# yxgeee/OpenIBL

Measured on NVIDIA H100. Metric: images_per_sec_extraction, higher is better.
Workload: dtype f32 (bf16x3 split on wgmma, fp32 accumulate)

## Files before the change

include/iblb200.h:

```cpp
#ifndef IBLB200_H_
#define IBLB200_H_

#include <stddef.h>
#include <stdint.h>

#ifdef __cplusplus
extern "C" {
#endif

#define IBLB200_ABI_VERSION 1

typedef enum ibl_status {
  IBL_OK = 0,
  IBL_ERR_BAD_ARG = 1,
  IBL_ERR_NOT_READY = 2,
  IBL_ERR_CUDA = 3,
  IBL_ERR_NO_DEVICE = 4,
  IBL_ERR_OOM = 5,
  IBL_ERR_UNSUPPORTED = 6
} ibl_status;

typedef struct ibl_engine ibl_engine;

#define IBL_OUT_VLAD 0x1u
// ... 91 lines not shown
                void* stream);

int ibl_debug_dist_flagged(ibl_engine* e, int* count, void* stream);
int ibl_debug_dist_path(ibl_engine* e, int* path);
int ibl_debug_knn_flagged(ibl_engine* e, int* count, void* stream);
int ibl_debug_rerank_workspace_bytes(ibl_engine* e, uint64_t* bytes);
int ibl_selftest_tc(ibl_engine* e, float* max_rel_err);

int ibl_debug_conv3x3(ibl_engine* e, const float* x_nhwc, int N, int H, int W, int cin,
                      const float* w_oihw, const float* bias, int cout, int relu, int pool, int mode,
                      int bn_override, float* y_nhwc, void* stream);

int ibl_debug_gemm_tn(ibl_engine* e, const float* A, const float* B, float* C, void* stream);
int ibl_debug_umma_strided(ibl_engine* e, const void* A, int rows, const void* B, int s0, int group_rows,
                           int base_mode, float* D, void* stream);
int ibl_debug_time_layer(ibl_engine* e, int layer, const float* x, int N, int H, int W, int bn_override,
                         int reps, float* ms_out);

#ifdef __cplusplus
}
#endif
#endif
```

openibl_b200/_cabi.py:

```python
from __future__ import annotations

import ctypes
import os
from ctypes import POINTER, c_char_p, c_double, c_float, c_int, c_int64, c_uint, c_uint64, c_void_p

_HERE = os.path.dirname(os.path.abspath(__file__))
LIB_PATH = os.path.join(_HERE, "lib", "libiblb200.so")

IBL_OK = 0
STATUS_NAMES = {0: "IBL_OK", 1: "IBL_ERR_BAD_ARG", 2: "IBL_ERR_NOT_READY", 3: "IBL_ERR_CUDA",
                4: "IBL_ERR_NO_DEVICE", 5: "IBL_ERR_OOM", 6: "IBL_ERR_UNSUPPORTED"}
OUT_VLAD, OUT_PCA, OUT_POOL = 0x1, 0x2, 0x4
CONV_SIMT_FP32, CONV_TC_BF16X3 = 0, 1

_P = c_void_p
SIGNATURES = {
    "ibl_abi_version": (c_int, []),
    "ibl_status_string": (c_char_p, [c_int]),
    "ibl_last_error": (c_char_p, []),
    "ibl_engine_create": (c_int, [c_int, POINTER(c_void_p)]),
    "ibl_engine_destroy": (c_int, [_P]),
    "ibl_engine_set_conv_mode": (c_int, [_P, c_int]),
    "ibl_engine_set_gemm_mode": (c_int, [_P, c_int]),
    "ibl_engine_get_conv_mode": (c_int, [_P, POINTER(c_int)]),
# ... 26 lines not shown
    "ibl_argsort_rows": (c_int, [_P, _P, c_int, c_int, _P, _P]),
    "ibl_topk_merge": (c_int, [_P, _P, _P, c_int, c_int, c_int, c_int, _P, _P, _P]),
    "ibl_l2dist_topk_host": (c_int, [_P, _P, c_int, _P, c_int, c_int, c_int, _P, _P, _P]),
    "ibl_knn_rowmax": (c_int, [_P, _P, c_int, c_int, c_int, c_int, c_int, _P, _P, _P, _P]),
    "ibl_rerank_topk": (c_int, [_P, _P, c_int, c_int, c_int, _P, _P, c_int, _P, c_int, c_int, c_float, _P, c_int,
                                c_int, _P, _P, _P]),
    "ibl_rerank_dense": (c_int, [_P, _P, _P, _P, c_int, c_int, c_int, c_int, c_double, _P, _P]),
    "ibl_debug_rerank_workspace_bytes": (c_int, [_P, POINTER(c_uint64)]),
    "ibl_debug_knn_flagged": (c_int, [_P, POINTER(c_int), _P]),
    "ibl_gemm_nt": (c_int, [_P, _P, c_int, _P, c_int, c_int, c_float, _P, c_int, _P]),
    "ibl_debug_dist_flagged": (c_int, [_P, POINTER(c_int), _P]),
    "ibl_debug_dist_path": (c_int, [_P, POINTER(c_int)]),
    "ibl_selftest_tc": (c_int, [_P, POINTER(c_float)]),
    "ibl_debug_gemm_tn": (c_int, [_P, _P, _P, _P, _P]),
    "ibl_debug_umma_strided": (c_int, [_P, _P, c_int, _P, c_int, c_int, c_int, _P, _P]),
    "ibl_debug_time_layer": (c_int, [_P, c_int, _P, c_int, c_int, c_int, c_int, c_int, POINTER(c_float)]),
    "ibl_debug_conv3x3": (c_int, [_P, _P, c_int, c_int, c_int, c_int, _P, _P, c_int, c_int, c_int, c_int,
                                  c_int, _P, _P]),
}

_lib = None


class IblError(RuntimeError):
    def __init__(self, status: int, where: str, detail: str):
        self.status = status
        super().__init__(f"{where}: {STATUS_NAMES.get(status, status)}: {detail}")


def load(build_if_missing: bool = True) -> ctypes.CDLL:
# ... 23 lines not shown
```

openibl_b200/csrc/common.cuh:

```cuda
#pragma once
#include <cuda_runtime.h>
#include <cuda_bf16.h>
#include <stdint.h>
#include <stdio.h>
#include <atomic>
#include <string>

#include "../../include/iblb200.h"

namespace ibl {

void set_last_error(const std::string& s);

#define IBL_CUDA_OK(expr)                                                          \
  do {                                                                             \
    cudaError_t _e = (expr);                                                       \
    if (_e != cudaSuccess) {                                                       \
      ::ibl::set_last_error(std::string(#expr) + ": " + cudaGetErrorString(_e) +   \
                            " (" __FILE__ ":" + std::to_string(__LINE__) + ")");   \
      return IBL_ERR_CUDA;                                                         \
    }                                                                              \
  } while (0)

#define IBL_RET(expr)                 \
// ... 72 lines not shown
                              const int* kk_h, int ksize_h, const int* bounds_v, const int* kk_v, int ksize_v,
                              uint8_t* tmp, uint8_t* out, cudaStream_t s, uint64_t* launches);
int launch_repack_weights_dgrad(const float* w_tck, int cout, int cin, __nv_bfloat16* w_hi, __nv_bfloat16* w_lo,
                                cudaStream_t s);
int launch_relu_mask_planes(const float* g, const float* y, size_t n, bool relu, __nv_bfloat16* hi, __nv_bfloat16* lo,
                            cudaStream_t s);
int launch_maxpool2x2_bwd(const float* x, const float* gy, int N, int H, int W, int C, float* gx, cudaStream_t s);
int wgrad_tc_splits(int N, int H, int W, int cin, int cout);
int launch_conv_wgrad_tc(const __nv_bfloat16* g_hi, const __nv_bfloat16* g_lo, const __nv_bfloat16* x_hi,
                         const __nv_bfloat16* x_lo, int N, int H, int W, int cin, int cout, float* part, int splits,
                         float* bpart, float* dw_oihw, float* db, cudaStream_t s);
int launch_conv1_1_wgrad(const float* x_nchw, const __nv_bfloat16* g_hi, const __nv_bfloat16* g_lo, int N, int H, int W,
                         float* part, float* dw_oihw, float* db, cudaStream_t s);
int launch_conv1_1_tc(const float* x_nchw, const float* w_oihw, const float* bias, int N, int H, int W,
                      __nv_bfloat16* y_hi, __nv_bfloat16* y_lo, cudaStream_t s);
int debug_gmma_strided(const void* A, int rows, const void* B, int s0, int group_rows, int base_mode, float* D,
                       cudaStream_t s);
int debug_gemm_tn(const float* A, const float* B, float* C, cudaStream_t s);
int netvlad_tc_units(int B, int S);
int launch_netvlad_tc(const __nv_bfloat16* x_hi, const __nv_bfloat16* x_lo, int B, int S,
                      const __nv_bfloat16* w_hi, const __nv_bfloat16* w_lo, const float* ssq, int ssq_parts,
                      const float* cent, bool normalize_input, float* part, float* asum_part, int* ticket,
                      float* vlad_raw, float* vlad_norm, cudaStream_t s);
int launch_global_maxpool_planes(const __nv_bfloat16* hi, const __nv_bfloat16* lo, int N, int S, int C, float* y,
                                 cudaStream_t s);

int dist_top16_max_runs(int n_valid);
int launch_dist_top16_tc(const __nv_bfloat16* q_hi, const __nv_bfloat16* q_lo, const float* qn, int m,
                         const __nv_bfloat16* d_hi, const __nv_bfloat16* d_lo, const float* dn, int n,
                         int n_valid, int K, float* cand_d, long long* cand_i, int max_runs, int* runs_out,
                         cudaStream_t s);
int launch_dist_dense_tc(const __nv_bfloat16* q_hi, const __nv_bfloat16* q_lo, const float* qn, int m,
// ... 72 lines not shown
```

openibl_b200/csrc/engine.cu:

```cuda
#include <stdlib.h>

#include <mutex>
#include <new>
#include <vector>

#include "common.cuh"

namespace ibl {

static thread_local std::string g_last_error;
void set_last_error(const std::string& s) { g_last_error = s; }
void tc_set_bn_override(int bn);

static const ConvLayer kVgg16[13] = {
    {3, 64, true, false},    {64, 64, true, true},
    {64, 128, true, false},  {128, 128, true, true},
    {128, 256, true, false}, {256, 256, true, false}, {256, 256, true, true},
    {256, 512, true, false}, {512, 512, true, false}, {512, 512, true, true},
    {512, 512, true, false}, {512, 512, true, false}, {512, 512, false, false}
};

struct DevBuf {
  void* p = nullptr;
  size_t cap = 0;
// ... 1185 lines not shown
  return rc;
}

int ibl_debug_gemm_tn(ibl_engine* e, const float* A, const float* B, float* C, void* stream) {
  IBL_REQUIRE(e && A && B && C, "null argument");
  DeviceGuard g(e->device);
  e->launches += 3;
  return debug_gemm_tn(A, B, C, S(stream));
}

int ibl_debug_umma_strided(ibl_engine* e, const void* A, int rows, const void* B, int s0, int group_rows,
                            int base_mode, float* D, void* stream) {
  IBL_REQUIRE(e && A && B && D, "null argument");
  DeviceGuard g(e->device);
  e->launches += 1;
  return debug_gmma_strided(A, rows, B, s0, group_rows, base_mode, D, S(stream));
}

int ibl_debug_time_layer(ibl_engine* e, int layer, const float* x, int N, int H, int W, int bn_override,
                         int reps, float* ms_out) {
  IBL_REQUIRE(e && x && ms_out && layer >= 0 && layer <= 12 && reps >= 1, "bad argument");
  if (!e->vgg_ready) { set_last_error("ibl_engine_set_vgg16 was not called"); return IBL_ERR_NOT_READY; }
  DeviceGuard g(e->device);
  const ConvLayer& L = kVgg16[layer];
  const size_t in_e = (size_t)N * H * W * L.cin;
  const int oh = L.pool ? H / 2 : H, ow = L.pool ? W / 2 : W;
  const size_t out_e = (size_t)N * oh * ow * L.cout;
  IBL_RET(e->act[0].ensure((in_e > out_e ? in_e : out_e) * 4));
  IBL_RET(e->act[1].ensure((in_e > out_e ? in_e : out_e) * 4));
  cudaEvent_t e0, e1;
  IBL_CUDA_OK(cudaEventCreate(&e0));
  IBL_CUDA_OK(cudaEventCreate(&e1));
  __nv_bfloat16* ih = e->act[0].as<__nv_bfloat16>();
  __nv_bfloat16* oh_ = e->act[1].as<__nv_bfloat16>();
  int rc = IBL_OK;
  if (layer > 0) rc = launch_f32_to_planes(x, in_e, ih, ih + in_e, nullptr);
  tc_set_bn_override(bn_override);
  for (int r = -1; r < reps && rc == IBL_OK; ++r) {
    if (r == 0) cudaEventRecord(e0, nullptr);
    if (layer == 0)
      rc = launch_conv1_1_tc(x, e->w0_oihw, e->conv[0].bias, N, H, W, oh_, oh_ + out_e, nullptr);
    else
      rc = launch_conv3x3_tc(ih, ih + in_e, e->conv[layer], N, H, W, L.cin, L.cout, L.relu, L.pool,
                             layer == 12 ? nullptr : oh_, layer == 12 ? nullptr : oh_ + out_e,
                             layer == 12 ? e->act[1].as<float>() : nullptr, nullptr);
  }
  tc_set_bn_override(0);
  cudaEventRecord(e1, nullptr);
  cudaError_t ce = cudaEventSynchronize(e1);
  float ms = 0.f;
  cudaEventElapsedTime(&ms, e0, e1);
  cudaEventDestroy(e0);
  cudaEventDestroy(e1);
  if (rc == IBL_OK && ce != cudaSuccess) { set_last_error(cudaGetErrorString(ce)); return IBL_ERR_CUDA; }
  *ms_out = ms / reps;
// ... 6 lines not shown
```

openibl_b200/csrc/tc_common.cuh:

```cuda
#pragma once
#include <cuda.h>
#include <cuda_runtime.h>
#include <stdint.h>

#include "wgmma.cuh"

namespace ibl {
namespace tc {

__device__ __forceinline__ uint32_t smem_u32(const void* p) {
  return static_cast<uint32_t>(__cvta_generic_to_shared(p));
}

__device__ __forceinline__ uint32_t warp_uniform(uint32_t v) { return __reduce_or_sync(0xffffffffu, v); }

__device__ __forceinline__ bool elect_one() {
  uint32_t pred;
  asm volatile(
      "{\n\t"
      ".reg .pred p;\n\t"
      "elect.sync _|p, 0xffffffff;\n\t"
      "selp.u32 %0, 1, 0, p;\n\t"
      "}"
      : "=r"(pred));
// ... 161 lines not shown
}
__device__ __forceinline__ uint64_t gmma_desc_mnmajor_sw128(uint32_t smem_addr, uint32_t lbo_bytes) {
  uint64_t d = 0;
  d |= (uint64_t)((smem_addr >> 4) & 0x3fffu);
  d |= (uint64_t)((lbo_bytes >> 4) & 0x3fffu) << 16;
  d |= (uint64_t)(1024u >> 4) << 32;
  d |= (uint64_t)1 << 62;
  return d;
}

__device__ __forceinline__ void wgmma_fence() { asm volatile("wgmma.fence.sync.aligned;" ::: "memory"); }
__device__ __forceinline__ void wgmma_commit() { asm volatile("wgmma.commit_group.sync.aligned;" ::: "memory"); }
template <int N>
__device__ __forceinline__ void wgmma_wait() { asm volatile("wgmma.wait_group.sync.aligned %0;" ::"n"(N) : "memory"); }

__device__ __forceinline__ void wg_sync() { asm volatile("bar.sync 1, 128;" ::: "memory"); }

template <int N>
struct Acc128 {
  float h[2][N / 2];
  template <bool F16 = false, int TA = 0, int TB = 0>
  __device__ __forceinline__ void mma(uint64_t a0, uint64_t a1, uint64_t b, uint32_t accumulate) {
    Wgmma<N, F16, TA, TB>::mma(h[0], a0, b, accumulate);
    Wgmma<N, F16, TA, TB>::mma(h[1], a1, b, accumulate);
  }
  __device__ __forceinline__ void fence_operands() {
#pragma unroll
    for (int j = 0; j < 2; ++j)
#pragma unroll
      for (int i = 0; i < N / 2; ++i) asm volatile("" : "+f"(h[j][i])::"memory");
  }
  __device__ __forceinline__ void rows32(int ch, float* stg, uint32_t (&raw)[32]) const;
};
constexpr int ACC_STG_PITCH = 36;
constexpr int ACC_STG_BYTES = 128 * ACC_STG_PITCH * 4;

template <int N>
__device__ __forceinline__ void Acc128<N>::rows32(int ch, float* stg, uint32_t (&raw)[32]) const {
  const int t = threadIdx.x & 127, w = t >> 5, l = t & 31;
  wg_sync();
#pragma unroll
  for (int j = 0; j < 2; ++j)
#pragma unroll
    for (int i = 0; i < 4; ++i) {
      const int r = 64 * j + 16 * w + (l >> 2), c = 8 * i + 2 * (l & 3);
      const float* f = &h[j][4 * (4 * ch + i)];
      *reinterpret_cast<float2*>(stg + r * ACC_STG_PITCH + c) = make_float2(f[0], f[1]);
      *reinterpret_cast<float2*>(stg + (r + 8) * ACC_STG_PITCH + c) = make_float2(f[2], f[3]);
    }
  wg_sync();
#pragma unroll
  for (int i = 0; i < 8; ++i) {
    const float4 v = *reinterpret_cast<const float4*>(stg + t * ACC_STG_PITCH + 4 * i);
    raw[4 * i] = __float_as_uint(v.x); raw[4 * i + 1] = __float_as_uint(v.y);
    raw[4 * i + 2] = __float_as_uint(v.z); raw[4 * i + 3] = __float_as_uint(v.w);
  }
}

typedef CUresult (*EncodeTiledFn)(CUtensorMap*, CUtensorMapDataType, cuuint32_t, void*,
                                  const cuuint64_t*, const cuuint64_t*, const cuuint32_t*,
                                  const cuuint32_t*, CUtensorMapInterleave, CUtensorMapSwizzle,
                                  CUtensorMapL2promotion, CUtensorMapFloatOOBfill);
EncodeTiledFn get_encode_tiled();

int make_tmap(CUtensorMap* out, CUtensorMapDataType dt, int rank, const void* base,
// ... 5 lines not shown
```

openibl_b200/csrc/tc_conv.cu:

```cuda
#include "common.cuh"
#include "tc_common.cuh"

namespace ibl {

using namespace tc;

namespace tc {
EncodeTiledFn get_encode_tiled() {
  static const EncodeTiledFn fn = []() -> EncodeTiledFn {
    void* p = nullptr;
    cudaDriverEntryPointQueryResult qres;
    if (cudaGetDriverEntryPoint("cuTensorMapEncodeTiled", &p, cudaEnableDefault, &qres) ==
            cudaSuccess &&
        qres == cudaDriverEntryPointSuccess)
      return reinterpret_cast<EncodeTiledFn>(p);
    return nullptr;
  }();
  return fn;
}

int make_tmap(CUtensorMap* out, CUtensorMapDataType dt, int rank, const void* base,
              const uint64_t* dims, const uint64_t* strides_bytes, const uint32_t* box, int swizzle_bytes) {
  EncodeTiledFn enc = get_encode_tiled();
  if (!enc) {
// ... 33 lines not shown
  const float* bias;
  __nv_bfloat16* y_hi;
  __nv_bfloat16* y_lo;
  float* y_f32;
  float* ssq;
  long long ssq_stride;
};

__device__ __forceinline__ uint32_t pack_bf16x2(float a, float b) {
  __nv_bfloat162 t = __floats2bfloat162_rn(a, b);
  return *reinterpret_cast<uint32_t*>(&t);
}

template <int BN>
__device__ __forceinline__ void conv_epilogue_tile(const ConvTcArgs& a, const Acc128<BN>& acc, float* stg, int img, int h0,
                                                   int w0, int n0, int nt, int r, int c, int TW) {
  const int h = h0 + r, w = w0 + c;
  bool valid;
  long long pix;
  if (a.pool) {
    const int OH = a.H >> 1, OW = a.W >> 1;
    const int oh = h >> 1, ow = w >> 1;
    valid = oh < OH && ow < OW && img < a.N;
    pix = ((long long)img * OH + oh) * OW + ow;
  } else {
    valid = h < a.H && w < a.W && img < a.N;
    pix = ((long long)img * a.H + h) * a.W + w;
  }
  float ssq_acc = 0.f;
#pragma unroll
  for (int ch = 0; ch < BN / 32; ++ch) {
    uint32_t raw[32];
    acc.rows32(ch, stg, raw);
    if (a.pool) {
      const bool s1 = (c & 1) != 0, s2 = (r & 1) != 0;
      float u[16];
#pragma unroll
      for (int j = 0; j < 16; ++j) {
        const float lo_h = __uint_as_float(raw[j]), hi_h = __uint_as_float(raw[j + 16]);
        const float got = __shfl_xor_sync(0xffffffffu, s1 ? lo_h : hi_h, 1);
        u[j] = fmaxf(s1 ? hi_h : lo_h, got);
      }
      float w8[8];
#pragma unroll
      for (int j = 0; j < 8; ++j) {
        const float got = __shfl_xor_sync(0xffffffffu, s2 ? u[j] : u[j + 8], TW);
        w8[j] = fmaxf(s2 ? u[j + 8] : u[j], got);
      }
      if (valid) {
        const int cbase = n0 + ch * 32 + (s1 ? 16 : 0) + (s2 ? 8 : 0);
        const float4 b0 = __ldg(reinterpret_cast<const float4*>(a.bias + cbase));
        const float4 b1 = __ldg(reinterpret_cast<const float4*>(a.bias + cbase) + 1);
        const float bb[8] = {b0.x, b0.y, b0.z, b0.w, b1.x, b1.y, b1.z, b1.w};
#pragma unroll
        for (int j = 0; j < 8; ++j) {
          w8[j] = w8[j] + bb[j];
          if (a.relu) w8[j] = fmaxf(w8[j], 0.f);
        }
        const long long off = pix * a.cout + cbase;
        if (a.y_f32) {
          float4* o = reinterpret_cast<float4*>(a.y_f32 + off);
// ... 55 lines not shown
        for (int j = 0; j < 4; ++j) {
          oh4[j] = make_uint4(hi[4 * j], hi[4 * j + 1], hi[4 * j + 2], hi[4 * j + 3]);
          ol4[j] = make_uint4(lo[4 * j], lo[4 * j + 1], lo[4 * j + 2], lo[4 * j + 3]);
        }
      }
    }
  }
  if (a.ssq && valid && !a.pool) a.ssq[(long long)nt * a.ssq_stride + pix] = ssq_acc;
}

constexpr int TC_BM = 128;
constexpr int TC_BK = 64;
constexpr int TC_A_BYTES = TC_BM * TC_BK * 2;

constexpr int TC_HALO_W = 10, TC_HALO_H = 18;
constexpr int TC_HALO_PLANE = 23 * 1024;
constexpr int TC_HALO_STAGE = 2 * TC_HALO_PLANE;

template <int BN, int STAGES, bool HALO = false, int NA = 0>
struct ConvTcSmem {
  static constexpr int B_BYTES = BN * TC_BK * 2;
  static constexpr int STAGE_BYTES = HALO ? 2 * B_BYTES : 2 * TC_A_BYTES + 2 * B_BYTES;
  static constexpr int A_RING = HALO ? NA * TC_HALO_STAGE : 0;
  static constexpr int BYTES = A_RING + STAGES * STAGE_BYTES + ACC_STG_BYTES + 1024  + 256 ;
};

template <int BN, int STAGES, bool HALO, int NA>
__global__ void __launch_bounds__(160, 1)
conv3x3_tc_kernel(const __grid_constant__ CUtensorMap tm_xhi, const __grid_constant__ CUtensorMap tm_xlo,
                  const __grid_constant__ CUtensorMap tm_whi, const __grid_constant__ CUtensorMap tm_wlo,
                  const ConvTcArgs a) {
  extern __shared__ __align__(1024) uint8_t smem_raw[];
  uint8_t* smem = reinterpret_cast<uint8_t*>((reinterpret_cast<uintptr_t>(smem_raw) + 1023) & ~uintptr_t(1023));
  using L = ConvTcSmem<BN, STAGES, HALO, NA>;
  constexpr int B_BYTES = L::B_BYTES;
  constexpr int STAGE_BYTES = L::STAGE_BYTES;
  constexpr int A_RING = L::A_RING;
  uint8_t* ring = smem + A_RING;
  float* stg = reinterpret_cast<float*>(ring + STAGES * STAGE_BYTES);
  uint64_t* bars = reinterpret_cast<uint64_t*>(ring + STAGES * STAGE_BYTES + ACC_STG_BYTES);
  uint64_t* full_bar = bars;
  uint64_t* empty_bar = bars + STAGES;
  uint64_t* afull_bar = bars + 2 * STAGES;
  uint64_t* aempty_bar = afull_bar + NA;

  const int warp = threadIdx.x >> 5, lane = threadIdx.x & 31;
  const int worker = (int)blockIdx.x;
  const int n_workers = (int)gridDim.x;
  if (warp == 4 && lane == 0) {
    tma_prefetch_desc(&tm_xhi);
    tma_prefetch_desc(&tm_xlo);
    tma_prefetch_desc(&tm_whi);
    tma_prefetch_desc(&tm_wlo);
    for (int i = 0; i < STAGES; ++i) {
      mbar_init(&full_bar[i], 1);
      mbar_init(&empty_bar[i], 4);
    }
    for (int i = 0; i < NA; ++i) {
      mbar_init(&afull_bar[i], 1);
      mbar_init(&aempty_bar[i], 4);
    }
    fence_barrier_init();
    fence_proxy_async();
  }
  __syncthreads();

  const int TW = 1 << a.tw_log2;
  const int kchunks = a.cin / TC_BK;
  const int kiters = 9 * kchunks;
  const int tiles_per_img = a.tiles_h * a.tiles_w;
  auto coords = [&](int tile, int& img, int& h0, int& w0, int& nt) {
    nt = tile % a.n_tiles;
    const int pt = tile / a.n_tiles;
    img = pt / tiles_per_img;
    const int rem = pt - img * tiles_per_img;
    h0 = (rem / a.tiles_w) * (TC_BM >> a.tw_log2);
    w0 = (rem % a.tiles_w) * TW;
  };

  if (warp == 4) {
    const uint32_t smem_a = warp_uniform(smem_u32(smem));
    const uint32_t ring_a = smem_a + A_RING;
    const uint32_t bars_a = ring_a + STAGES * STAGE_BYTES + ACC_STG_BYTES;
    const uint32_t full_a = bars_a, empty_a = bars_a + 8 * STAGES;
    const uint32_t afull_a = bars_a + 16 * STAGES, aempty_a = afull_a + 8 * NA;
    auto load_w = [&](uint32_t st, uint32_t fb, int c0, int n0, int tap) {
      tma_load_3d_a(st, &tm_whi, fb, c0, n0, tap);
      tma_load_3d_a(st + B_BYTES, &tm_wlo, fb, c0, n0, tap);
    };
    int stage = 0;
    uint32_t phase = 0;
    if constexpr (HALO) {
      auto try_wait_warp = [&](uint32_t bar, uint32_t parity) -> bool {
        uint32_t ok = 0;
        if (lane == 0) {
          asm volatile(
              "{\n\t"
              ".reg .pred p;\n\t"
// ... 6 lines not shown
        }
        return warp_uniform(ok) != 0;
      };
      int astage = 0;
      uint32_t aphase = 0;
      int tA = worker, kcA = 0, tB = worker, kcB = 0, tapB = 0;
      while (tB < a.total_tiles) {
        const uint32_t as_u = warp_uniform((uint32_t)astage);
        if (tA < a.total_tiles && try_wait_warp(aempty_a + 8 * as_u, aphase ^ 1)) {
          int img, h0, w0, nt;
          coords(tA, img, h0, w0, nt);
          img = (int)warp_uniform((uint32_t)img); h0 = (int)warp_uniform((uint32_t)h0);
          w0 = (int)warp_uniform((uint32_t)w0);
          const int c0 = (int)warp_uniform((uint32_t)(kcA * TC_BK));
          const uint32_t sa = smem_a + as_u * TC_HALO_STAGE;
          constexpr uint32_t kHaloBytes = 2u * TC_HALO_W * TC_HALO_H * 128u;
          if (elect_one()) {
            mbar_arrive_expect_tx_a(afull_a + 8 * as_u, kHaloBytes);
            tma_load_4d_a(sa, &tm_xhi, afull_a + 8 * as_u, c0, w0 - 1, h0 - 1, img);
            tma_load_4d_a(sa + TC_HALO_PLANE, &tm_xlo, afull_a + 8 * as_u, c0, w0 - 1, h0 - 1, img);
          }
          __syncwarp();
          if (++astage == NA) { astage = 0; aphase ^= 1; }
          if (++kcA == kchunks) { kcA = 0; tA += n_workers; }
          continue;
        }
        const uint32_t st_u = warp_uniform((uint32_t)stage);
        if (try_wait_warp(empty_a + 8 * st_u, phase ^ 1)) {
          int img, h0, w0, nt;
          coords(tB, img, h0, w0, nt);
          const int n0 = (int)warp_uniform((uint32_t)(nt * BN));
// ... 22 lines not shown
        const int kh = tap / 3 - 1, kw = tap % 3 - 1;
        const uint32_t st_u = warp_uniform((uint32_t)stage);
        mbar_wait_warp_a(empty_a + 8 * st_u, phase ^ 1);
        const uint32_t st = smem_a + st_u * STAGE_BYTES;
        if (elect_one()) {
          const uint32_t fb = full_a + 8 * st_u;
          mbar_arrive_expect_tx_a(fb, STAGE_BYTES);
          tma_load_4d_a(st, &tm_xhi, fb, c0, w0 + kw, h0 + kh, img);
          tma_load_4d_a(st + TC_A_BYTES, &tm_xlo, fb, c0, w0 + kw, h0 + kh, img);
          load_w(st + 2 * TC_A_BYTES, fb, c0, n0, tap);
        }
        __syncwarp();
        if (++stage == STAGES) { stage = 0; phase ^= 1; }
      }
    }
  } else {
    const int m = threadIdx.x;
    const int r = m >> a.tw_log2, c = m & (TW - 1);
    const uint32_t smem_a = smem_u32(smem);
    const uint32_t ring_a = smem_a + A_RING;
    int stage = 0, astage = 0;
    uint32_t phase = 0, aphase = 0;
    (void)ring_a; (void)astage; (void)aphase;
    auto release_w = [&](int st) {
      if (lane == 0) mbar_arrive(&empty_bar[st]);
    };
    for (int tile = worker; tile < a.total_tiles; tile += n_workers) {
      int img, h0, w0, nt;
      coords(tile, img, h0, w0, nt);
      Acc128<BN> acc;
      int prev = -1;
      if constexpr (HALO) {
        constexpr uint64_t kHaloDesc = ((uint64_t)1 << 16) | ((uint64_t)((TC_HALO_W * 128) >> 4) << 32) | ((uint64_t)1 << 62);
        constexpr uint64_t kHalf = 8 * TC_HALO_W * 128 / 16;
        for (int kc = 0; kc < kchunks; ++kc) {
          mbar_wait(&afull_bar[astage], aphase);
          const uint32_t ha = smem_a + astage * TC_HALO_STAGE;
          for (int tap = 0; tap < 9; ++tap) {
            mbar_wait(&full_bar[stage], phase);
            const uint32_t toff = (uint32_t)((tap / 3) * TC_HALO_W + tap % 3) * 128u;
            const uint64_t a_hi = kHaloDesc | (uint64_t)(((ha + toff) >> 4) & 0x3fffu);
            const uint64_t a_lo = kHaloDesc | (uint64_t)(((ha + TC_HALO_PLANE + toff) >> 4) & 0x3fffu);
            const uint32_t sb = ring_a + stage * STAGE_BYTES;
            const uint64_t b_hi = gmma_desc_kmajor_sw128(sb), b_lo = gmma_desc_kmajor_sw128(sb + B_BYTES);
            wgmma_fence();
#pragma unroll
            for (int k = 0; k < TC_BK / 16; ++k) {
              const uint64_t ko = (uint64_t)(k * 2);
              acc.mma(a_lo + ko, a_lo + kHalf + ko, b_hi + ko, (kc > 0 || tap > 0 || k > 0) ? 1u : 0u);
              acc.mma(a_hi + ko, a_hi + kHalf + ko, b_lo + ko, 1u);
              acc.mma(a_hi + ko, a_hi + kHalf + ko, b_hi + ko, 1u);
            }
            wgmma_commit();
            if (tap < 8) {
              wgmma_wait<1>();
              if (prev >= 0) release_w(prev);
              prev = stage;
            } else {
              wgmma_wait<0>();
              if (prev >= 0) release_w(prev);
              release_w(stage);
              if (lane == 0) mbar_arrive(&aempty_bar[astage]);
              prev = -1;
            }
            if (++stage == STAGES) { stage = 0; phase ^= 1; }
          }
          if (++astage == NA) { astage = 0; aphase ^= 1; }
        }
      } else
      for (int kit = 0; kit < kiters; ++kit) {
        mbar_wait(&full_bar[stage], phase);
        const uint32_t sa = ring_a + stage * STAGE_BYTES;
        const uint64_t a_hi = gmma_desc_kmajor_sw128(sa), a_lo = gmma_desc_kmajor_sw128(sa + TC_A_BYTES);
        const uint64_t b_hi = gmma_desc_kmajor_sw128(sa + 2 * TC_A_BYTES);
        const uint64_t b_lo = gmma_desc_kmajor_sw128(sa + 2 * TC_A_BYTES + B_BYTES);
        constexpr uint64_t kHalf = (TC_BM / 2) * 128 / 16;
        wgmma_fence();
#pragma unroll
        for (int k = 0; k < TC_BK / 16; ++k) {
          const uint64_t ko = (uint64_t)(k * 2);
          acc.mma(a_lo + ko, a_lo + kHalf + ko, b_hi + ko, (kit > 0 || k > 0) ? 1u : 0u);
          acc.mma(a_hi + ko, a_hi + kHalf + ko, b_lo + ko, 1u);
          acc.mma(a_hi + ko, a_hi + kHalf + ko, b_hi + ko, 1u);
        }
        wgmma_commit();
        wgmma_wait<1>();
        if (prev >= 0) release_w(prev);
        prev = stage;
        if (++stage == STAGES) { stage = 0; phase ^= 1; }
      }
      wgmma_wait<0>();
      acc.fence_operands();
      if (prev >= 0) release_w(prev);
      conv_epilogue_tile<BN>(a, acc, stg, img, h0, w0, nt * BN, nt, r, c, TW);
    }
  }
  __syncthreads();
}

template <int BN, int STAGES, bool HALO = false, int NA = 0>
static int launch_tc_variant(const CUtensorMap& xhi, const CUtensorMap& xlo, const CUtensorMap& whi,
                             const CUtensorMap& wlo, const ConvTcArgs& a, cudaStream_t s) {
  constexpr int smem = ConvTcSmem<BN, STAGES, HALO, NA>::BYTES;
  static_assert(smem <= 232448, "shared-memory budget");
  static DeviceOnce attr_done;
  if (!attr_done.done()) {
    IBL_CUDA_OK(cudaFuncSetAttribute(conv3x3_tc_kernel<BN, STAGES, HALO, NA>, cudaFuncAttributeMaxDynamicSharedMemorySize, smem));
    attr_done.mark();
  }
  const int sms = device_sm_count();
  const int grid = a.total_tiles < sms ? a.total_tiles : sms;
  conv3x3_tc_kernel<BN, STAGES, HALO, NA><<<grid, 160, smem, s>>>(xhi, xlo, whi, wlo, a);
  IBL_CUDA_OK(cudaGetLastError());
  return IBL_OK;
}

static int g_tc_bn_override = 0;
void tc_set_bn_override(int bn) { g_tc_bn_override = bn; }

int launch_conv3x3_tc(const __nv_bfloat16* x_hi, const __nv_bfloat16* x_lo, const ConvParams& p,
                      int N, int H, int W, int cin, int cout, bool relu, bool pool,
                      __nv_bfloat16* y_hi, __nv_bfloat16* y_lo, float* y_f32, cudaStream_t s, float* ssq,
                      int* ssq_parts) {
  IBL_REQUIRE(cin % 64 == 0 && cout % 64 == 0, "tensor-core conv needs Cin%64==0 and Cout%64==0");
  IBL_REQUIRE(p.w_hi && p.w_lo, "tensor-core conv: weights were not re-laid-out");
  IBL_REQUIRE(H >= 1 && W >= 1 && N >= 1, "empty conv input");
  ConvTcArgs a{};
  a.N = N; a.H = H; a.W = W; a.cin = cin; a.cout = cout;
  auto waste = [&](int tw) {
    int th = 128 / tw;
    return (long long)cdiv(W, tw) * tw * cdiv(H, th) * th;
  };
  a.tw_log2 = (waste(16) <= waste(8)) ? 4 : 3;
  const int TW = 1 << a.tw_log2, TH = 128 / TW;
  a.tiles_w = cdiv(W, TW);
  a.tiles_h = cdiv(H, TH);
  int bn = cout % 128 == 0 ? 128 : 64;
  if (g_tc_bn_override && cout % g_tc_bn_override == 0 && (g_tc_bn_override == 64 || g_tc_bn_override == 128))
    bn = g_tc_bn_override;
  const bool halo = bn == 128;
  if (halo) {
    a.tw_log2 = 3;
    a.tiles_w = cdiv(W, 8);
    a.tiles_h = cdiv(H, 16);
  }
  a.n_tiles = cout / bn;
  a.total_tiles = (int)((long long)N * a.tiles_h * a.tiles_w * a.n_tiles);
  a.relu = relu; a.pool = pool;
  a.bias = p.bias; a.y_hi = y_hi; a.y_lo = y_lo; a.y_f32 = y_f32;
  a.ssq = pool ? nullptr : ssq;
  a.ssq_stride = (long long)N * H * W;
  if (ssq_parts) *ssq_parts = a.n_tiles;

  CUtensorMap m_xhi, m_xlo, m_whi, m_wlo;
  {
    uint64_t dims[4] = {(uint64_t)cin, (uint64_t)W, (uint64_t)H, (uint64_t)N};
    uint64_t str[3] = {(uint64_t)cin * 2, (uint64_t)W * cin * 2, (uint64_t)H * W * cin * 2};
    uint32_t box[4] = {64, (uint32_t)(halo ? TC_HALO_W : TW), (uint32_t)(halo ? TC_HALO_H : TH), 1};
    IBL_RET(make_tmap(&m_xhi, CU_TENSOR_MAP_DATA_TYPE_BFLOAT16, 4, x_hi, dims, str, box));
    IBL_RET(make_tmap(&m_xlo, CU_TENSOR_MAP_DATA_TYPE_BFLOAT16, 4, x_lo, dims, str, box));
  }
  {
    uint64_t dims[3] = {(uint64_t)cin, (uint64_t)cout, 9};
    uint64_t str[2] = {(uint64_t)cin * 2, (uint64_t)cout * cin * 2};
    uint32_t box[3] = {64, (uint32_t)bn, 1};
    IBL_RET(make_tmap(&m_whi, CU_TENSOR_MAP_DATA_TYPE_BFLOAT16, 3, p.w_hi, dims, str, box));
    IBL_RET(make_tmap(&m_wlo, CU_TENSOR_MAP_DATA_TYPE_BFLOAT16, 3, p.w_lo, dims, str, box));
  }
  if (halo) return launch_tc_variant<128, 3, true, 2>(m_xhi, m_xlo, m_whi, m_wlo, a, s);
  return launch_tc_variant<64, 4>(m_xhi, m_xlo, m_whi, m_wlo, a, s);
}

struct Conv1FusedArgs {
// ... 327 lines not shown
```

openibl_b200/csrc/tc_probe.cu:

```cuda
#include "common.cuh"
#include "tc_common.cuh"

namespace ibl {

using namespace tc;

__device__ __forceinline__ uint64_t probe_desc(uint32_t a_addr, uint32_t sbo, int base_mode) {
  uint64_t d = 0;
  d |= (uint64_t)((a_addr >> 4) & 0x3fffu);
  d |= (uint64_t)1 << 16;
  d |= (uint64_t)((sbo >> 4) & 0x3fffu) << 32;
  if (base_mode == 1) d |= (uint64_t)((a_addr >> 7) & 7u) << 49;
  d |= (uint64_t)1 << 62;
  return d;
}

__global__ void __launch_bounds__(128, 1)
gmma_strided_probe_kernel(const __grid_constant__ CUtensorMap tm_a, const __grid_constant__ CUtensorMap tm_b,
                          int rows, int s0, int group_rows, int base_mode, float* __restrict__ D) {
  extern __shared__ __align__(1024) uint8_t smem_raw[];
  uint8_t* smem = reinterpret_cast<uint8_t*>((reinterpret_cast<uintptr_t>(smem_raw) + 1023) & ~uintptr_t(1023));
  uint8_t* a_sm = smem;
  uint8_t* b_sm = smem + 32768;
  float* stg = reinterpret_cast<float*>(smem + 32768 + 8192);
  uint64_t* bars = reinterpret_cast<uint64_t*>(smem + 32768 + 8192 + ACC_STG_BYTES);
  if (threadIdx.x == 0) {
    mbar_init(&bars[0], 1);
    fence_barrier_init();
    fence_proxy_async();
  }
  __syncthreads();
  if (threadIdx.x == 0) {
    mbar_arrive_expect_tx(&bars[0], rows * 128 + 8192);
    tma_load_2d(a_sm, &tm_a, &bars[0], 0, 0);
    tma_load_2d(b_sm, &tm_b, &bars[0], 0, 0);
  }
  mbar_wait(&bars[0], 0);
  const uint32_t sbo = (uint32_t)group_rows * 128u;
  const uint32_t a0 = smem_u32(a_sm) + (uint32_t)s0 * 128u;
  const uint32_t a1 = a0 + 8u * sbo;
  const uint64_t da0 = probe_desc(a0, sbo, base_mode), da1 = probe_desc(a1, sbo, base_mode);
  const uint64_t db = gmma_desc_kmajor_sw128(smem_u32(b_sm));
  Acc128<64> acc;
  wgmma_fence();
#pragma unroll
  for (int k = 0; k < 4; ++k)
    acc.mma(da0 + (uint64_t)(k * 2), da1 + (uint64_t)(k * 2), db + (uint64_t)(k * 2), k > 0 ? 1u : 0u);
  wgmma_commit();
  wgmma_wait<0>();
  acc.fence_operands();
  float* o = D + (size_t)threadIdx.x * 64;
#pragma unroll
  for (int ch = 0; ch < 2; ++ch) {
    uint32_t r[32];
    acc.rows32(ch, stg, r);
#pragma unroll
    for (int j = 0; j < 32; ++j) o[ch * 32 + j] = __uint_as_float(r[j]);
  }
}

int debug_gmma_strided(const void* A, int rows, const void* B, int s0, int group_rows, int base_mode, float* D,
                       cudaStream_t s) {
  IBL_REQUIRE(rows >= 8 && rows <= 256 && s0 >= 0 && group_rows >= 8 && s0 + 15 * group_rows + 8 <= rows,
              "probe view does not fit the halo tile");
  CUtensorMap ma, mb;
  {
    uint64_t dims[2] = {64, (uint64_t)rows};
    uint64_t str[1] = {128};
    uint32_t box[2] = {64, (uint32_t)rows};
    IBL_RET(make_tmap(&ma, CU_TENSOR_MAP_DATA_TYPE_BFLOAT16, 2, A, dims, str, box));
  }
  {
    uint64_t dims[2] = {64, 64};
    uint64_t str[1] = {128};
    uint32_t box[2] = {64, 64};
    IBL_RET(make_tmap(&mb, CU_TENSOR_MAP_DATA_TYPE_BFLOAT16, 2, B, dims, str, box));
  }
  const int smem = 32768 + 8192 + ACC_STG_BYTES + 1024 + 64;
  static DeviceOnce attr_done;
  if (!attr_done.done()) {
    IBL_CUDA_OK(cudaFuncSetAttribute(gmma_strided_probe_kernel, cudaFuncAttributeMaxDynamicSharedMemorySize, smem));
    attr_done.mark();
  }
  gmma_strided_probe_kernel<<<1, 128, smem, s>>>(ma, mb, rows, s0, group_rows, base_mode, D);
  IBL_CUDA_OK(cudaGetLastError());
  return IBL_OK;
}

}
```

Before: 818.8.

## Use two ping-pong consumer warpgroups with register reallocation in halo conv kernel

The halo-tiled conv3x3 wgmma kernel now uses 384 threads: one producer warpgroup that gives up registers via setmaxnreg, and two consumer warpgroups that alternate tiles. An order barrier hands the MMA pipe from one to the other, so one warpgroup's epilogue can overlap the other's MMAs. Each consumer gets its own staging buffer and named barrier. The halo tile shape now follows TW/TH instead of a forced 8x16, with matching descriptor and pixel mapping changes. This costs extra shared memory and adds more complex phase bookkeeping.

```diff
diff --git a/include/iblb200.h b/include/iblb200.h
--- a/include/iblb200.h
+++ b/include/iblb200.h
@@ -129,6 +129,8 @@
 int ibl_debug_gemm_tn(ibl_engine* e, const float* A, const float* B, float* C, void* stream);
 int ibl_debug_umma_strided(ibl_engine* e, const void* A, int rows, const void* B, int s0, int group_rows,
                            int base_mode, float* D, void* stream);
+int ibl_debug_umma_halo_view(ibl_engine* e, const void* A, int rows, const void* B, int s0, int group_rows,
+                             int half_rows, float* D, void* stream);
 int ibl_debug_time_layer(ibl_engine* e, int layer, const float* x, int N, int H, int W, int bn_override,
                          int reps, float* ms_out);
 
diff --git a/openibl_b200/_cabi.py b/openibl_b200/_cabi.py
--- a/openibl_b200/_cabi.py
+++ b/openibl_b200/_cabi.py
@@ -64,6 +64,7 @@
     "ibl_selftest_tc": (c_int, [_P, POINTER(c_float)]),
     "ibl_debug_gemm_tn": (c_int, [_P, _P, _P, _P, _P]),
     "ibl_debug_umma_strided": (c_int, [_P, _P, c_int, _P, c_int, c_int, c_int, _P, _P]),
+    "ibl_debug_umma_halo_view": (c_int, [_P, _P, c_int, _P, c_int, c_int, c_int, _P, _P]),
     "ibl_debug_time_layer": (c_int, [_P, c_int, _P, c_int, c_int, c_int, c_int, c_int, POINTER(c_float)]),
     "ibl_debug_conv3x3": (c_int, [_P, _P, c_int, c_int, c_int, c_int, _P, _P, c_int, c_int, c_int, c_int,
                                   c_int, _P, _P]),
diff --git a/openibl_b200/csrc/common.cuh b/openibl_b200/csrc/common.cuh
--- a/openibl_b200/csrc/common.cuh
+++ b/openibl_b200/csrc/common.cuh
@@ -110,8 +110,8 @@
                          float* part, float* dw_oihw, float* db, cudaStream_t s);
 int launch_conv1_1_tc(const float* x_nchw, const float* w_oihw, const float* bias, int N, int H, int W,
                       __nv_bfloat16* y_hi, __nv_bfloat16* y_lo, cudaStream_t s);
-int debug_gmma_strided(const void* A, int rows, const void* B, int s0, int group_rows, int base_mode, float* D,
-                       cudaStream_t s);
+int debug_gmma_strided(const void* A, int rows, const void* B, int s0, int group_rows, int half_rows, int base_mode,
+                       float* D, cudaStream_t s);
 int debug_gemm_tn(const float* A, const float* B, float* C, cudaStream_t s);
 int netvlad_tc_units(int B, int S);
 int launch_netvlad_tc(const __nv_bfloat16* x_hi, const __nv_bfloat16* x_lo, int B, int S,
diff --git a/openibl_b200/csrc/engine.cu b/openibl_b200/csrc/engine.cu
--- a/openibl_b200/csrc/engine.cu
+++ b/openibl_b200/csrc/engine.cu
@@ -1223,15 +1223,24 @@
   IBL_REQUIRE(e && A && B && D, "null argument");
   DeviceGuard g(e->device);
   e->launches += 1;
-  return debug_gmma_strided(A, rows, B, s0, group_rows, base_mode, D, S(stream));
+  return debug_gmma_strided(A, rows, B, s0, group_rows, 8 * group_rows, base_mode, D, S(stream));
+}
+
+int ibl_debug_umma_halo_view(ibl_engine* e, const void* A, int rows, const void* B, int s0, int group_rows,
+                             int half_rows, float* D, void* stream) {
+  IBL_REQUIRE(e && A && B && D, "null argument");
+  DeviceGuard g(e->device);
+  e->launches += 1;
+  return debug_gmma_strided(A, rows, B, s0, group_rows, half_rows, 0, D, S(stream));
 }
 
 int ibl_debug_time_layer(ibl_engine* e, int layer, const float* x, int N, int H, int W, int bn_override,
                          int reps, float* ms_out) {
-  IBL_REQUIRE(e && x && ms_out && layer >= 0 && layer <= 12 && reps >= 1, "bad argument");
+  IBL_REQUIRE(e && x && ms_out && layer >= -1 && layer <= 12 && reps >= 1, "bad argument");
   if (!e->vgg_ready) { set_last_error("ibl_engine_set_vgg16 was not called"); return IBL_ERR_NOT_READY; }
   DeviceGuard g(e->device);
-  const ConvLayer& L = kVgg16[layer];
+  const bool fused1 = layer < 0;
+  const ConvLayer& L = kVgg16[fused1 ? 1 : layer];
   const size_t in_e = (size_t)N * H * W * L.cin;
   const int oh = L.pool ? H / 2 : H, ow = L.pool ? W / 2 : W;
   const size_t out_e = (size_t)N * oh * ow * L.cout;
@@ -1247,7 +1256,9 @@
   tc_set_bn_override(bn_override);
   for (int r = -1; r < reps && rc == IBL_OK; ++r) {
     if (r == 0) cudaEventRecord(e0, nullptr);
-    if (layer == 0)
+    if (fused1)
+      rc = launch_conv1_fused_tc(x, e->w0_oihw, e->conv[0].bias, e->conv[1], N, H, W, oh_, oh_ + out_e, nullptr);
+    else if (layer == 0)
       rc = launch_conv1_1_tc(x, e->w0_oihw, e->conv[0].bias, N, H, W, oh_, oh_ + out_e, nullptr);
     else
       rc = launch_conv3x3_tc(ih, ih + in_e, e->conv[layer], N, H, W, L.cin, L.cout, L.relu, L.pool,
diff --git a/openibl_b200/csrc/tc_common.cuh b/openibl_b200/csrc/tc_common.cuh
--- a/openibl_b200/csrc/tc_common.cuh
+++ b/openibl_b200/csrc/tc_common.cuh
@@ -199,7 +199,12 @@
 template <int N>
 __device__ __forceinline__ void wgmma_wait() { asm volatile("wgmma.wait_group.sync.aligned %0;" ::"n"(N) : "memory"); }
 
-__device__ __forceinline__ void wg_sync() { asm volatile("bar.sync 1, 128;" ::: "memory"); }
+__device__ __forceinline__ void wg_sync(int id = 1) { asm volatile("bar.sync %0, 128;" ::"r"(id) : "memory"); }
+
+template <int N>
+__device__ __forceinline__ void setmaxnreg_dec() { asm volatile("setmaxnreg.dec.sync.aligned.u32 %0;" ::"n"(N)); }
+template <int N>
+__device__ __forceinline__ void setmaxnreg_inc() { asm volatile("setmaxnreg.inc.sync.aligned.u32 %0;" ::"n"(N)); }
 
 template <int N>
 struct Acc128 {
@@ -215,15 +220,15 @@
 #pragma unroll
       for (int i = 0; i < N / 2; ++i) asm volatile("" : "+f"(h[j][i])::"memory");
   }
-  __device__ __forceinline__ void rows32(int ch, float* stg, uint32_t (&raw)[32]) const;
+  __device__ __forceinline__ void rows32(int ch, float* stg, uint32_t (&raw)[32], int bar = 1) const;
 };
 constexpr int ACC_STG_PITCH = 36;
 constexpr int ACC_STG_BYTES = 128 * ACC_STG_PITCH * 4;
 
 template <int N>
-__device__ __forceinline__ void Acc128<N>::rows32(int ch, float* stg, uint32_t (&raw)[32]) const {
+__device__ __forceinline__ void Acc128<N>::rows32(int ch, float* stg, uint32_t (&raw)[32], int bar) const {
   const int t = threadIdx.x & 127, w = t >> 5, l = t & 31;
-  wg_sync();
+  wg_sync(bar);
 #pragma unroll
   for (int j = 0; j < 2; ++j)
 #pragma unroll
@@ -233,7 +238,7 @@
       *reinterpret_cast<float2*>(stg + r * ACC_STG_PITCH + c) = make_float2(f[0], f[1]);
       *reinterpret_cast<float2*>(stg + (r + 8) * ACC_STG_PITCH + c) = make_float2(f[2], f[3]);
     }
-  wg_sync();
+  wg_sync(bar);
 #pragma unroll
   for (int i = 0; i < 8; ++i) {
     const float4 v = *reinterpret_cast<const float4*>(stg + t * ACC_STG_PITCH + 4 * i);
diff --git a/openibl_b200/csrc/tc_conv.cu b/openibl_b200/csrc/tc_conv.cu
--- a/openibl_b200/csrc/tc_conv.cu
+++ b/openibl_b200/csrc/tc_conv.cu
@@ -71,7 +71,7 @@
 
 template <int BN>
 __device__ __forceinline__ void conv_epilogue_tile(const ConvTcArgs& a, const Acc128<BN>& acc, float* stg, int img, int h0,
-                                                   int w0, int n0, int nt, int r, int c, int TW) {
+                                                   int w0, int n0, int nt, int r, int c, int dr_lanes, int bar = 1) {
   const int h = h0 + r, w = w0 + c;
   bool valid;
   long long pix;
@@ -88,7 +88,7 @@
 #pragma unroll
   for (int ch = 0; ch < BN / 32; ++ch) {
     uint32_t raw[32];
-    acc.rows32(ch, stg, raw);
+    acc.rows32(ch, stg, raw, bar);
     if (a.pool) {
       const bool s1 = (c & 1) != 0, s2 = (r & 1) != 0;
       float u[16];
@@ -101,7 +101,7 @@
       float w8[8];
 #pragma unroll
       for (int j = 0; j < 8; ++j) {
-        const float got = __shfl_xor_sync(0xffffffffu, s2 ? u[j] : u[j + 8], TW);
+        const float got = __shfl_xor_sync(0xffffffffu, s2 ? u[j] : u[j + 8], dr_lanes);
         w8[j] = fmaxf(s2 ? u[j + 8] : u[j], got);
       }
       if (valid) {
@@ -187,19 +187,23 @@
 constexpr int TC_A_BYTES = TC_BM * TC_BK * 2;
 
 constexpr int TC_HALO_W = 10, TC_HALO_H = 18;
+constexpr int TC_HALO_ROWS = TC_HALO_W * TC_HALO_H;
 constexpr int TC_HALO_PLANE = 23 * 1024;
 constexpr int TC_HALO_STAGE = 2 * TC_HALO_PLANE;
 
 template <int BN, int STAGES, bool HALO = false, int NA = 0>
 struct ConvTcSmem {
+  static constexpr int THREADS = HALO ? 384 : 160;
+  static constexpr int CONSUMERS = HALO ? 2 : 1;
   static constexpr int B_BYTES = BN * TC_BK * 2;
   static constexpr int STAGE_BYTES = HALO ? 2 * B_BYTES : 2 * TC_A_BYTES + 2 * B_BYTES;
   static constexpr int A_RING = HALO ? NA * TC_HALO_STAGE : 0;
-  static constexpr int BYTES = A_RING + STAGES * STAGE_BYTES + ACC_STG_BYTES + 1024  + 256 ;
+  static constexpr int STG = CONSUMERS * ACC_STG_BYTES;
+  static constexpr int BYTES = A_RING + STAGES * STAGE_BYTES + STG + 1024  + 256 ;
 };
 
 template <int BN, int STAGES, bool HALO, int NA>
-__global__ void __launch_bounds__(160, 1)
+__global__ void __launch_bounds__(ConvTcSmem<BN, STAGES, HALO, NA>::THREADS, 1)
 conv3x3_tc_kernel(const __grid_constant__ CUtensorMap tm_xhi, const __grid_constant__ CUtensorMap tm_xlo,
                   const __grid_constant__ CUtensorMap tm_whi, const __grid_constant__ CUtensorMap tm_wlo,
                   const ConvTcArgs a) {
@@ -211,16 +215,18 @@
   constexpr int A_RING = L::A_RING;
   uint8_t* ring = smem + A_RING;
   float* stg = reinterpret_cast<float*>(ring + STAGES * STAGE_BYTES);
-  uint64_t* bars = reinterpret_cast<uint64_t*>(ring + STAGES * STAGE_BYTES + ACC_STG_BYTES);
+  uint64_t* bars = reinterpret_cast<uint64_t*>(ring + STAGES * STAGE_BYTES + L::STG);
   uint64_t* full_bar = bars;
   uint64_t* empty_bar = bars + STAGES;
   uint64_t* afull_bar = bars + 2 * STAGES;
   uint64_t* aempty_bar = afull_bar + NA;
+  uint64_t* order_bar = aempty_bar + NA;
 
   const int warp = threadIdx.x >> 5, lane = threadIdx.x & 31;
   const int worker = (int)blockIdx.x;
   const int n_workers = (int)gridDim.x;
-  if (warp == 4 && lane == 0) {
+  const int producer_warp = HALO ? 0 : 4;
+  if (warp == producer_warp && lane == 0) {
     tma_prefetch_desc(&tm_xhi);
     tma_prefetch_desc(&tm_xlo);
     tma_prefetch_desc(&tm_whi);
@@ -232,6 +238,10 @@
     for (int i = 0; i < NA; ++i) {
       mbar_init(&afull_bar[i], 1);
       mbar_init(&aempty_bar[i], 4);
+    }
+    if (HALO) {
+      mbar_init(&order_bar[0], 4);
+      mbar_init(&order_bar[1], 4);
     }
     fence_barrier_init();
     fence_proxy_async();
@@ -251,10 +261,11 @@
     w0 = (rem % a.tiles_w) * TW;
   };
 
-  if (warp == 4) {
+  if (HALO && warp < 4) setmaxnreg_dec<40>();
+  if (warp == producer_warp) {
     const uint32_t smem_a = warp_uniform(smem_u32(smem));
     const uint32_t ring_a = smem_a + A_RING;
-    const uint32_t bars_a = ring_a + STAGES * STAGE_BYTES + ACC_STG_BYTES;
+    const uint32_t bars_a = ring_a + STAGES * STAGE_BYTES + L::STG;
     const uint32_t full_a = bars_a, empty_a = bars_a + 8 * STAGES;
     const uint32_t afull_a = bars_a + 16 * STAGES, aempty_a = afull_a + 8 * NA;
     auto load_w = [&](uint32_t st, uint32_t fb, int c0, int n0, int tap) {
@@ -291,7 +302,7 @@
           w0 = (int)warp_uniform((uint32_t)w0);
           const int c0 = (int)warp_uniform((uint32_t)(kcA * TC_BK));
           const uint32_t sa = smem_a + as_u * TC_HALO_STAGE;
-          constexpr uint32_t kHaloBytes = 2u * TC_HALO_W * TC_HALO_H * 128u;
+          constexpr uint32_t kHaloBytes = 2u * TC_HALO_ROWS * 128u;
           if (elect_one()) {
             mbar_arrive_expect_tx_a(afull_a + 8 * as_u, kHaloBytes);
             tma_load_4d_a(sa, &tm_xhi, afull_a + 8 * as_u, c0, w0 - 1, h0 - 1, img);
@@ -344,60 +355,79 @@
         if (++stage == STAGES) { stage = 0; phase ^= 1; }
       }
     }
-  } else {
-    const int m = threadIdx.x;
-    const int r = m >> a.tw_log2, c = m & (TW - 1);
+  } else if (!HALO || warp >= 4) {
     const uint32_t smem_a = smem_u32(smem);
     const uint32_t ring_a = smem_a + A_RING;
-    int stage = 0, astage = 0;
-    uint32_t phase = 0, aphase = 0;
-    (void)ring_a; (void)astage; (void)aphase;
     auto release_w = [&](int st) {
       if (lane == 0) mbar_arrive(&empty_bar[st]);
     };
+    if constexpr (HALO) {
+    setmaxnreg_inc<232>();
+    const int cw = warp / 4 - 1;
+    const int bar = 1 + cw;
+    float* my_stg = stg + cw * (ACC_STG_BYTES / 4);
+    const int m = threadIdx.x & 127;
+    const int r = TW == 16 ? (m >> 3) & 7 : m >> 3;
+    const int c = TW == 16 ? ((m >> 6) << 3) | (m & 7) : m & 7;
+    const uint32_t halo_w = (uint32_t)TW + 2;
+    const uint64_t halo_desc = ((uint64_t)1 << 16) | ((uint64_t)((halo_w * 128) >> 4) << 32) | ((uint64_t)1 << 62);
+    const uint64_t a_half = (TW == 16 ? 8u : 8u * halo_w) * 128u / 16u;
+    for (int i = cw; worker + i * n_workers < a.total_tiles; i += 2) {
+      int img, h0, w0, nt;
+      coords(worker + i * n_workers, img, h0, w0, nt);
+      int astage = (i * kchunks) % NA, stage = (i * kiters) % STAGES;
+      uint32_t aphase = (uint32_t)((i * kchunks) / NA) & 1u, phase = (uint32_t)((i * kiters) / STAGES) & 1u;
+      if (i > 0) mbar_wait(&order_bar[cw], (uint32_t)((i - 1) >> 1) & 1u);
+      Acc128<BN> acc;
+      int prev = -1, prev_a = -1;
+      for (int kc = 0; kc < kchunks; ++kc) {
+        mbar_wait(&afull_bar[astage], aphase);
+        const uint32_t ha = smem_a + astage * TC_HALO_STAGE;
+        for (int tap = 0; tap < 9; ++tap) {
+          mbar_wait(&full_bar[stage], phase);
+          const uint32_t toff = ((uint32_t)(tap / 3) * halo_w + (uint32_t)(tap % 3)) * 128u;
+          const uint64_t a_hi = halo_desc | (uint64_t)(((ha + toff) >> 4) & 0x3fffu);
+          const uint64_t a_lo = halo_desc | (uint64_t)(((ha + TC_HALO_PLANE + toff) >> 4) & 0x3fffu);
+          const uint32_t sb = ring_a + stage * STAGE_BYTES;
+          const uint64_t b_hi = gmma_desc_kmajor_sw128(sb), b_lo = gmma_desc_kmajor_sw128(sb + B_BYTES);
+          wgmma_fence();
+#pragma unroll
+          for (int k = 0; k < TC_BK / 16; ++k) {
+            const uint64_t ko = (uint64_t)(k * 2);
+            acc.mma(a_lo + ko, a_lo + a_half + ko, b_hi + ko, (kc > 0 || tap > 0 || k > 0) ? 1u : 0u);
+            acc.mma(a_hi + ko, a_hi + a_half + ko, b_lo + ko, 1u);
+            acc.mma(a_hi + ko, a_hi + a_half + ko, b_hi + ko, 1u);
+          }
+          wgmma_commit();
+          if (kc == kchunks - 1 && tap == 8 && lane == 0) mbar_arrive(&order_bar[cw ^ 1]);
+          wgmma_wait<1>();
+          if (prev >= 0) release_w(prev);
+          if (prev_a >= 0) {
+            if (lane == 0) mbar_arrive(&aempty_bar[prev_a]);
+            prev_a = -1;
+          }
+          prev = stage;
+          if (++stage == STAGES) { stage = 0; phase ^= 1; }
+        }
+        prev_a = astage;
+        if (++astage == NA) { astage = 0; aphase ^= 1; }
+      }
+      wgmma_wait<0>();
+      acc.fence_operands();
+      release_w(prev);
+      if (lane == 0) mbar_arrive(&aempty_bar[prev_a]);
+      conv_epilogue_tile<BN>(a, acc, my_stg, img, h0, w0, nt * BN, nt, r, c, 8, bar);
+    }
+    } else {
+    const int m = threadIdx.x;
+    const int r = m >> a.tw_log2, c = m & (TW - 1);
+    int stage = 0;
+    uint32_t phase = 0;
     for (int tile = worker; tile < a.total_tiles; tile += n_workers) {
       int img, h0, w0, nt;
       coords(tile, img, h0, w0, nt);
       Acc128<BN> acc;
       int prev = -1;
-      if constexpr (HALO) {
-        constexpr uint64_t kHaloDesc = ((uint64_t)1 << 16) | ((uint64_t)((TC_HALO_W * 128) >> 4) << 32) | ((uint64_t)1 << 62);
-        constexpr uint64_t kHalf = 8 * TC_HALO_W * 128 / 16;
-        for (int kc = 0; kc < kchunks; ++kc) {
-          mbar_wait(&afull_bar[astage], aphase);
-          const uint32_t ha = smem_a + astage * TC_HALO_STAGE;
-          for (int tap = 0; tap < 9; ++tap) {
-            mbar_wait(&full_bar[stage], phase);
-            const uint32_t toff = (uint32_t)((tap / 3) * TC_HALO_W + tap % 3) * 128u;
-            const uint64_t a_hi = kHaloDesc | (uint64_t)(((ha + toff) >> 4) & 0x3fffu);
-            const uint64_t a_lo = kHaloDesc | (uint64_t)(((ha + TC_HALO_PLANE + toff) >> 4) & 0x3fffu);
-            const uint32_t sb = ring_a + stage * STAGE_BYTES;
-            const uint64_t b_hi = gmma_desc_kmajor_sw128(sb), b_lo = gmma_desc_kmajor_sw128(sb + B_BYTES);
-            wgmma_fence();
-#pragma unroll
-            for (int k = 0; k < TC_BK / 16; ++k) {
-              const uint64_t ko = (uint64_t)(k * 2);
-              acc.mma(a_lo + ko, a_lo + kHalf + ko, b_hi + ko, (kc > 0 || tap > 0 || k > 0) ? 1u : 0u);
-              acc.mma(a_hi + ko, a_hi + kHalf + ko, b_lo + ko, 1u);
-              acc.mma(a_hi + ko, a_hi + kHalf + ko, b_hi + ko, 1u);
-            }
-            wgmma_commit();
-            if (tap < 8) {
-              wgmma_wait<1>();
-              if (prev >= 0) release_w(prev);
-              prev = stage;
-            } else {
-              wgmma_wait<0>();
-              if (prev >= 0) release_w(prev);
-              release_w(stage);
-              if (lane == 0) mbar_arrive(&aempty_bar[astage]);
-              prev = -1;
-            }
-            if (++stage == STAGES) { stage = 0; phase ^= 1; }
-          }
-          if (++astage == NA) { astage = 0; aphase ^= 1; }
-        }
-      } else
       for (int kit = 0; kit < kiters; ++kit) {
         mbar_wait(&full_bar[stage], phase);
         const uint32_t sa = ring_a + stage * STAGE_BYTES;
@@ -423,6 +453,7 @@
       acc.fence_operands();
       if (prev >= 0) release_w(prev);
       conv_epilogue_tile<BN>(a, acc, stg, img, h0, w0, nt * BN, nt, r, c, TW);
+    }
     }
   }
   __syncthreads();
@@ -440,7 +471,7 @@
   }
   const int sms = device_sm_count();
   const int grid = a.total_tiles < sms ? a.total_tiles : sms;
-  conv3x3_tc_kernel<BN, STAGES, HALO, NA><<<grid, 160, smem, s>>>(xhi, xlo, whi, wlo, a);
+  conv3x3_tc_kernel<BN, STAGES, HALO, NA><<<grid, ConvTcSmem<BN, STAGES, HALO, NA>::THREADS, smem, s>>>(xhi, xlo, whi, wlo, a);
   IBL_CUDA_OK(cudaGetLastError());
   return IBL_OK;
 }
@@ -469,11 +500,6 @@
   if (g_tc_bn_override && cout % g_tc_bn_override == 0 && (g_tc_bn_override == 64 || g_tc_bn_override == 128))
     bn = g_tc_bn_override;
   const bool halo = bn == 128;
-  if (halo) {
-    a.tw_log2 = 3;
-    a.tiles_w = cdiv(W, 8);
-    a.tiles_h = cdiv(H, 16);
-  }
   a.n_tiles = cout / bn;
   a.total_tiles = (int)((long long)N * a.tiles_h * a.tiles_w * a.n_tiles);
   a.relu = relu; a.pool = pool;
@@ -486,7 +512,7 @@
   {
     uint64_t dims[4] = {(uint64_t)cin, (uint64_t)W, (uint64_t)H, (uint64_t)N};
     uint64_t str[3] = {(uint64_t)cin * 2, (uint64_t)W * cin * 2, (uint64_t)H * W * cin * 2};
-    uint32_t box[4] = {64, (uint32_t)(halo ? TC_HALO_W : TW), (uint32_t)(halo ? TC_HALO_H : TH), 1};
+    uint32_t box[4] = {64, (uint32_t)(halo ? TW + 2 : TW), (uint32_t)(halo ? TH + 2 : TH), 1};
     IBL_RET(make_tmap(&m_xhi, CU_TENSOR_MAP_DATA_TYPE_BFLOAT16, 4, x_hi, dims, str, box));
     IBL_RET(make_tmap(&m_xlo, CU_TENSOR_MAP_DATA_TYPE_BFLOAT16, 4, x_lo, dims, str, box));
   }
diff --git a/openibl_b200/csrc/tc_probe.cu b/openibl_b200/csrc/tc_probe.cu
--- a/openibl_b200/csrc/tc_probe.cu
+++ b/openibl_b200/csrc/tc_probe.cu
@@ -17,7 +17,7 @@
 
 __global__ void __launch_bounds__(128, 1)
 gmma_strided_probe_kernel(const __grid_constant__ CUtensorMap tm_a, const __grid_constant__ CUtensorMap tm_b,
-                          int rows, int s0, int group_rows, int base_mode, float* __restrict__ D) {
+                          int rows, int s0, int group_rows, int half_rows, int base_mode, float* __restrict__ D) {
   extern __shared__ __align__(1024) uint8_t smem_raw[];
   uint8_t* smem = reinterpret_cast<uint8_t*>((reinterpret_cast<uintptr_t>(smem_raw) + 1023) & ~uintptr_t(1023));
   uint8_t* a_sm = smem;
@@ -38,7 +38,7 @@
   mbar_wait(&bars[0], 0);
   const uint32_t sbo = (uint32_t)group_rows * 128u;
   const uint32_t a0 = smem_u32(a_sm) + (uint32_t)s0 * 128u;
-  const uint32_t a1 = a0 + 8u * sbo;
+  const uint32_t a1 = a0 + (uint32_t)half_rows * 128u;
   const uint64_t da0 = probe_desc(a0, sbo, base_mode), da1 = probe_desc(a1, sbo, base_mode);
   const uint64_t db = gmma_desc_kmajor_sw128(smem_u32(b_sm));
   Acc128<64> acc;
@@ -59,9 +59,10 @@
   }
 }
 
-int debug_gmma_strided(const void* A, int rows, const void* B, int s0, int group_rows, int base_mode, float* D,
-                       cudaStream_t s) {
-  IBL_REQUIRE(rows >= 8 && rows <= 256 && s0 >= 0 && group_rows >= 8 && s0 + 15 * group_rows + 8 <= rows,
+int debug_gmma_strided(const void* A, int rows, const void* B, int s0, int group_rows, int half_rows, int base_mode,
+                       float* D, cudaStream_t s) {
+  IBL_REQUIRE(rows >= 8 && rows <= 256 && s0 >= 0 && group_rows >= 8 && half_rows >= 0 &&
+                  s0 + half_rows + 7 * group_rows + 8 <= rows,
               "probe view does not fit the halo tile");
   CUtensorMap ma, mb;
   {
@@ -82,7 +83,7 @@
     IBL_CUDA_OK(cudaFuncSetAttribute(gmma_strided_probe_kernel, cudaFuncAttributeMaxDynamicSharedMemorySize, smem));
     attr_done.mark();
   }
-  gmma_strided_probe_kernel<<<1, 128, smem, s>>>(ma, mb, rows, s0, group_rows, base_mode, D);
+  gmma_strided_probe_kernel<<<1, 128, smem, s>>>(ma, mb, rows, s0, group_rows, half_rows, base_mode, D);
   IBL_CUDA_OK(cudaGetLastError());
   return IBL_OK;
 }
```

Result: faster. 889.6 (median of 6 runs) (+8.6%).
